# seanrjohnson/protein_gibbs_sampler

Hardware: AMD Instinct MI355X
Metric: sampled positions/sec (whole node), ESM-1b L=256 B=256 Gibbs (higher is better)
Workload: dtype bf16; 1 GPU; ESM_sampler ESM-1b (33 layers, d=1280) Gibbs: 256 chains in total, 256 per GPU x L=256 (T=258), P=25 positions per chain per iteration, mask=True top_k=0 temperature=1.0 burnin=inf; bf16 MFMA operands, fp32 accumulate + fp32 residual stream; synthetic weights N(0,0.025), embeddings N(0,0.3), LayerNorm jitter 0.1 (logit std ~10); global_batch=256, seq_len=256, parallelism=chains sharded 1-way (contiguous blocks), 1 RCCL all-gather at the end, n_layers=33

## Files before the change

protein_gibbs_sampler_amd/csrc/api_dbg.hip:

```cpp
#include <math.h>
#include <string.h>

#include <algorithm>
#include <vector>

#include "engine.h"
#include "gemm_epilogue.h"

using namespace pg;

namespace {
struct Dbg {
  int prev = -1;
  bool bad = false;
  std::vector<void*> bufs;
  Dbg() { (void)hipGetDevice(&prev); }
  ~Dbg() {
    for (void* p : bufs) (void)hipFree(p);
    if (prev >= 0) (void)hipSetDevice(prev);
  }
  int open(int device) {
    int n = 0;
    if (hipGetDeviceCount(&n) != hipSuccess || n == 0) return fail(PG_ERR_NO_DEVICE, "no HIP device visible");
    if (device < 0 || device >= n) return fail(PG_ERR_INVALID, "bad device ordinal");
// ... 83 lines not shown
  for (int i = 0; i < iters; ++i)
    if ((rc = launch())) return rc;
  PG_HIP(hipEventRecord(ev.b, nullptr));
  PG_HIP(hipEventSynchronize(ev.b));
  float ms = 0;
  PG_HIP(hipEventElapsedTime(&ms, ev.a, ev.b));
  *avg_ms = ms / iters;
  return PG_OK;
}
void dbg_noted_text(char* plan, int plan_bytes) {
  if (plan && plan_bytes > 0) snprintf(plan, (size_t)plan_bytes, "%s", noted_kernels().c_str());
}

template <typename Launch>
int dbg_attention_run(Dbg& s, int precision, bool strict, const float* qkv, float* ctx, int64_t M, int d, const int32_t* tok, char* plan,
                      int plan_bytes, Launch&& launch) {
  const float* dq = s.up(qkv, (size_t)M * 3 * d);
  const int32_t* dtok = s.up(tok, (size_t)M);
  bf16_t* bq = strict ? nullptr : s.alloc<bf16_t>((size_t)M * 3 * d);
  bf16_t* out = s.alloc<bf16_t>((size_t)M * d * (strict ? 3 : 1));
  float* wide = strict ? nullptr : s.alloc<float>((size_t)M * d);
  int rc = s.check();
  if (rc) return rc;
  clear_noted_kernels();
  if (!strict && (rc = to16(precision, dq, bq, M * 3 * d))) return rc;
  if ((rc = launch(dq, bq, out, dtok))) return rc;
  dbg_noted_text(plan, plan_bytes);
  return strict ? split3_rows_to_host(out, ctx, M, d) : down16(s, precision, out, wide, ctx, M * d);
}
}

extern "C" {

int pg_dbg_gemm(int device, int precision, const float* x, const float* w, const float* bias, float* out, int M, int N,
                int K, int epi) {
  return pg_dbg_gemm_v(device, precision, x, w, bias, out, M, N, K, epi, -1, -1, M, nullptr, 0);
}

int pg_dbg_gemm_v(int device, int precision, const float* x, const float* w, const float* bias, float* out, int M, int N, int K, int epi,
                  int variant, int have_ws, int m_live, char* plan, int plan_bytes) {
  if (plan && plan_bytes > 0) plan[0] = 0;
  int rc = dbg_precision("pg_dbg_gemm", precision, true);
  if (rc) return rc;
// ... 110 lines not shown
  }, iters, avg_ms);
}

int pg_dbg_gemm_plan(int M, int N, int K, int epi, int variant, int have_ws, int m_live, int n_cu, char* buf, int buf_bytes) {
  if (!buf || buf_bytes < 2 || M < 1 || N < 1 || K < 1 || n_cu < 1) return fail(PG_ERR_INVALID, "pg_dbg_gemm_plan: bad argument");
  std::string text;
  gemm_plan_text(M, N, K, epi, variant, have_ws != 0, m_live, n_cu, &text);
  snprintf(buf, (size_t)buf_bytes, "%s", text.c_str());
  return PG_OK;
}

int pg_dbg_attention_plan(int kind, int precision, int64_t n_seq_or_B, int T_or_C, int R, int H, int head_dim, int has_pad, int has_bias,
                          int row_step, int order_bh, int n_cu, char* buf, int buf_bytes) {
  const int rc = dbg_precision("pg_dbg_attention_plan", precision, true);
  if (rc) return rc;
  if (!buf || buf_bytes < 2 || (kind != 0 && kind != 1) || n_seq_or_B < 1 || H < 1 || n_cu < 1 || (kind == 1 && (R < 1 || n_seq_or_B > 0x7fffffff)))
    return fail(PG_ERR_INVALID, "pg_dbg_attention_plan: bad argument");
  const bool strict = precision == PG_PREC_FP32;
  std::string text;
  if (kind == 0 && strict) attention_f32_plan_text(n_seq_or_B, T_or_C, H, head_dim, has_pad != 0, has_bias != 0, row_step, &text);
  else if (kind == 0) attention_plan_text(n_seq_or_B, T_or_C, H, head_dim, has_pad != 0, has_bias != 0, row_step, n_cu, &text);
  else if (strict) msa_row_f32_plan_text((int)n_seq_or_B, R, T_or_C, H, has_pad != 0, &text);
  else msa_row_plan_text((int)n_seq_or_B, R, T_or_C, H, order_bh, &text);
  snprintf(buf, (size_t)buf_bytes, "%s", text.c_str());
  return PG_OK;
}

int pg_dbg_rowln_bench(int device, int M, int K, int iters, double* ms, double* max_diff) {
  if (!ms || M < 256 || K % 64 || K < 128 || iters < 1) return fail(PG_ERR_INVALID, "pg_dbg_rowln_bench: bad argument");
  Dbg d;
  int rc = d.open(device);
  if (rc) return rc;
  const int N = 768, Mp = round_up(M, kRowPad);
  const size_t n_f = (size_t)std::max(Mp, N) * std::max(K, N);
  const std::vector<float> hbuf = lcg_uniform(n_f + 5, 4242u);
// ... 115 lines not shown
  if ((rc = s.open(device))) return rc;
  const int d = H * head_dim;
  const bool strict = precision == PG_PREC_FP32;
  float* bias32 = bias_k ? s.alloc<float>((size_t)2 * d) : nullptr;
  if (bias_k) s.put(bias32, bias_k, (size_t)d), s.put(bias32 + d, bias_v, (size_t)d);
  bf16_t* bias16 = bias_k && !strict ? s.alloc<bf16_t>((size_t)2 * d) : nullptr;
  return dbg_attention_run(s, precision, strict, qkv, ctx, (int64_t)B * T, d, key_tok, plan, plan_bytes,
                           [&](const float* dq, const bf16_t* bq, bf16_t* out, const int32_t* dtok) {
    const SeqLayout chain = {1, T, 0, 1};
    if (strict) return launch_attention_f32(nullptr, dq, out, d, B, T, H, 3 * d, 3 * d, d, 2 * d, chain, dtok, pad_idx, bias32, head_dim);
    const int rc16 = bias_k ? to16(precision, bias32, bias16, 2 * d) : PG_OK;
    return rc16 ? rc16 : OPS(launch_attention_bf16, nullptr, bq, out, B, T, H, 3 * d, d, d, 2 * d, dtok, pad_idx, bias16, head_dim);
  });
}

int pg_dbg_layernorm_operand(int device, int precision, const float* x, const float* gamma, const float* beta, float* y, int M, int d,
                             float eps) {
  int rc = dbg_precision("pg_dbg_layernorm_operand", precision, true);
  if (rc) return rc;
  if (!x || !gamma || !beta || !y || M < 1 || d < 32 || d % 32) return fail(PG_ERR_INVALID, "pg_dbg_layernorm_operand: bad argument");
  Dbg s;
  if ((rc = s.open(device))) return rc;
  const bool split = precision == PG_PREC_FP32;
  const float* dx = s.up(x, (size_t)M * d);
  const float* dg = s.up(gamma, (size_t)d);
  const float* dbt = s.up(beta, (size_t)d);
  float* dy = s.alloc<float>((size_t)M * d);
  bf16_t* h = s.alloc<bf16_t>((size_t)M * d * (split ? 3 : 1));
  if ((rc = s.check())) return rc;
  if ((rc = OPS(launch_layernorm_bf16, nullptr, dx, dg, dbt, h, M, d, eps, split, 0, 0, true))) return rc;
// ... 261 lines not shown
```

protein_gibbs_sampler_amd/csrc/attention.hip:

```cpp
#include <stdlib.h>

#include "attn_frag.h"

PG_OPS_BEGIN


#ifdef PG_ATT_PROF
__device__ unsigned long long* pg_att_prof;
#define PG_T(slot, i)                                                                                              \
  do {                                                                                                             \
    if ((slot) < 8 && (threadIdx.x & 63) == 0)                                                                     \
      pg_att_prof[(((size_t)blockIdx.x * 4 + (threadIdx.x >> 6)) * 8 + (slot)) * 8 + (i)] = __builtin_readcyclecounter(); \
  } while (0)
#else
#define PG_T(slot, i)
#endif

constexpr int attention_occupancy(int maxkb, int hd, bool pad = false) {
  return hd == 128 ? (maxkb <= 8 || (maxkb == 10 && !pad) ? 2 : 1) : hd == 64 ? (maxkb <= 18 ? 2 : 1) : 2;
}
constexpr int attention_resident(int kb, int hd) {
  return hd == 128 ? (kb <= 4 ? 4 : (kb <= 6 ? 3 : (kb <= 10 ? 2 : 1))) : hd == 64 ? (kb <= 20 ? 2 : 1) : (kb <= 20 ? 4 : (kb <= 26 ? 3 : 2));
}
template <int MAXKB, bool PADMASK, bool BIASKV = false, bool SPLIT = false, int HD = 64>
__global__ __launch_bounds__(256, attention_occupancy(MAXKB, HD, PADMASK)) void attention_kernel(const bf16_t* __restrict__ qkv, bf16_t* __restrict__ ctx, int T,
                                                       int H, int ld_qkv_, int ld_ctx_, int k_off, int v_off,
                                                       SeqLayout sl, const int32_t* __restrict__ key_tok, int pad_idx,
                                                       const bf16_t* __restrict__ bias_kv, int split_from = 0, int split = 1) {
  constexpr int ROW = HD * 2, NKK = HD / 32, NDB = HD / 16;
  __shared__ __attribute__((aligned(16))) char smem[2 * MAXKB * 16 * ROW + (PADMASK ? MAXKB * 16 : 0)];
  char* Ks = smem;
  char* Vs = smem + MAXKB * 16 * ROW;
  char* padf = smem + 2 * MAXKB * 16 * ROW;

  const int tid = threadIdx.x, lane = tid & 63, wave = tid >> 6;
  PG_T(7, 0);
  int pair = blockIdx.x, qb_first = wave, qb_step = 4;
  if (SPLIT && (int)blockIdx.x >= split_from) {
    const int u = blockIdx.x - split_from;
    pair = split_from + u / split;
    qb_first = u % split + split * wave;
    qb_step = 4 * split;
  }
// ... 2 lines not shown
  const size_t ld_qkv = (size_t)ld_qkv_ * sl.row_step, ld_ctx = (size_t)ld_ctx_ * sl.row_step;
  const bf16_t* base = qkv + row0 * ld_qkv_ + h * HD;
  const int Tk = T + (BIASKV ? 1 : 0);
  constexpr int nkc = MAXKB / 2;

  stage_kv<MAXKB * 16, 256, BIASKV, HD>(Ks, Vs, tid, base, ld_qkv, k_off, v_off, 0, T, bias_kv + h * HD, bias_kv + (H + h) * HD);
  if (PADMASK) {
    for (int key = tid; key < MAXKB * 16; key += 256)
      padf[key] = (key < T && key_tok[row0 + (size_t)key * sl.row_step] == pad_idx) ? 1 : 0;
  }
  PG_T(7, 1);
  __syncthreads();
  PG_T(7, 2);

  const int fr = lane & 15, fq = lane >> 4;
  const int nqb = (T + 15) >> 4;
  bf16x8 qf[NKK], qn[NKK];
  auto load_q = [&](int qb, bf16x8 (&dst)[NKK]) {
    int qrow = qb * 16 + fr;
    if (qrow >= T) qrow = T - 1;
#pragma unroll
    for (int kk = 0; kk < NKK; ++kk) dst[kk] = *(const bf16x8*)(base + (size_t)qrow * ld_qkv + kk * 32 + fq * 8);
  };
  if (qb_first < nqb) load_q(qb_first, qf);
  for (int qb = qb_first; qb < nqb; qb += qb_step) {
    if (qb + qb_step < nqb) load_q(qb + qb_step, qn);
    PG_T(qb >> 2, 0);

    f32x4 st[MAXKB];
    {
      constexpr int CH = HD == 128 ? 2 : (MAXKB % 6 == 0) ? 6 : (MAXKB % 4 == 0 ? 4 : 2);
      bf16x8 kbuf[2][CH][NKK];
      auto load_chunk = [&](int ch, bf16x8 (&dst)[CH][NKK]) {
#pragma unroll
        for (int u = 0; u < CH; ++u) {
#if defined(PG_ATT_PROF) && PG_ATT_ABL == 1
          const int krow = (ch * CH + (u > 0 ? 0 : u)) * 16 + fr;
// ... 65 lines not shown
      };
      load_v(0, vbuf[0]);
      if (nkc > 1) load_v(1, vbuf[1]);
#pragma unroll
      for (int c = 0; c < nkc; ++c) {
        if (c + 2 < nkc) load_v(c + 2, vbuf[(c + 2) % 3]);
        const bf16x8 pf = p_frag(st[2 * c], st[2 * c + 1]);
        __builtin_amdgcn_sched_barrier(0);
#pragma unroll
        for (int db = 0; db < NDB; ++db) o[db] = mfma_op16(vbuf[c % 3][db].v, pf, o[db]);
        __builtin_amdgcn_sched_barrier(0);
      }
    }
    PG_T(qb >> 2, 3);
    const int q = qb * 16 + fr;
    if (q < T) store_ctx(o, inv, ctx + row0 * ld_ctx_ + (size_t)q * ld_ctx + h * HD + fq * 4);
    qf[0] = qn[0];
    if constexpr (NKK == 2) qf[1] = qn[1];
    if constexpr (NKK == 4) { qf[1] = qn[1]; qf[2] = qn[2]; qf[3] = qn[3]; }
    PG_T(qb >> 2, 4);
  }
  PG_T(7, 3);
}

template <int MAXKB, int OCC, bool PADMASK, bool BIASKV, int HD = 64>
__global__ __launch_bounds__(256, OCC) void attention_long_kernel(const bf16_t* __restrict__ qkv, bf16_t* __restrict__ ctx, int T,
                                                               int H, int ld_qkv_, int ld_ctx_, int k_off, int v_off,
                                                               SeqLayout sl, int n_qchunk, const int32_t* __restrict__ key_tok_,
                                                               int pad_idx, const bf16_t* __restrict__ bias_kv_) {
  const int32_t* __restrict__ key_tok = PADMASK ? key_tok_ : nullptr;
  const bf16_t* __restrict__ bias_kv = BIASKV ? bias_kv_ : nullptr;
// ... 178 lines not shown

int launch_attention_seq_bf16(hipStream_t s, const bf16_t* qkv, bf16_t* ctx, int64_t n_seq, int T, int H, int ld_qkv,
                              int ld_ctx, int k_off, int v_off, SeqLayout sl, const int32_t* key_tok, int pad_idx,
                              const bf16_t* bias_kv, int head_dim) {
  const AttentionPlan p = plan_attention(n_seq, T, H, head_dim, key_tok != nullptr, bias_kv != nullptr, sl.row_step, device_cu_count());
  if (!p.error.empty()) return fail(1, p.error);
  if (!p.grid) return 0;
  note_kernel(plan_text(p).c_str());
  auto launch = [&](auto hd) {
    constexpr int HD = decltype(hd)::value;
    if (!p.whole)
      return launch_long<HD>(p.pad, p.bias, dim3(p.grid), s, qkv, ctx, T, H, ld_qkv, ld_ctx, k_off, v_off, sl, p.n_qchunk, key_tok,
                             pad_idx, bias_kv);
    visit_rung(p.kb, [&](auto kb) {
      launch_rung<decltype(kb)::value, HD>(p.pad, p.bias, p.split > 1, dim3(p.grid), s, qkv, ctx, T, H, ld_qkv, ld_ctx, k_off, v_off,
                                           sl, key_tok, pad_idx, bias_kv, p.split_from, p.split);
    });
  };
  if (head_dim == 64) launch(std::integral_constant<int, 64>{});
  else if (head_dim == 128) launch(std::integral_constant<int, 128>{});
  else launch(std::integral_constant<int, 32>{});
  PG_HIP(hipGetLastError());
  return 0;
}

int launch_attention_bf16(hipStream_t s, const bf16_t* qkv, bf16_t* ctx, int B, int T, int H, int ld_qkv, int ld_ctx,
                          int k_off, int v_off, const int32_t* key_tok, int pad_idx, const bf16_t* bias_kv, int head_dim) {
  SeqLayout sl = {1, T, 0, 1};
  return launch_attention_seq_bf16(s, qkv, ctx, B, T, H, ld_qkv, ld_ctx, k_off, v_off, sl, key_tok, pad_idx, bias_kv, head_dim);
}

PG_OPS_END
```

protein_gibbs_sampler_amd/csrc/engine.h:

```cpp
#pragma once
#include <map>
#include <string>
#include <vector>

#include "kernels.h"

namespace pg {

#define OPS(fn, ...) (precision == PG_PREC_F16 ? opf16::fn(__VA_ARGS__) : opbf16::fn(__VA_ARGS__))

struct DevBuf {
  void* p = nullptr;
  size_t bytes = 0;
  int ensure(size_t need, hipStream_t s);
  void release();
  template <typename T> T* as() const { return (T*)p; }
};

struct Prof {
  struct Rec { int cls; hipEvent_t a, b; std::string kernels; };
  bool on = false;
  std::vector<Rec> recs;
  std::vector<hipEvent_t> pool;
  size_t used = 0;
// ... 32 lines not shown
  pg_model_config cfg;
  int device = 0;
  int precision = 0;
  hipStream_t own_stream = nullptr, stream = nullptr;
  std::vector<void*> owned;

  float *embed = nullptr, *pos = nullptr, *msa_pos = nullptr, *embed_out = nullptr;
  float embed_scale() const { return cfg.arch == PG_ARCH_ESM1 ? sqrtf((float)cfg.d_model) : 1.0f; }
  LnW ln_before, ln_after, head_ln;
  DenseW head_dense;
  float* head_bias = nullptr;
  std::vector<EsmLayer> esm_layers;
  std::vector<MsaLayer> msa_layers;

  DevBuf x, h, qkv, ctx, ffn, sel_h, sel_g, logits, d_tokens, d_idx, d_samp_tok, d_samp_logits, d_rowmap, scratch;
  DevBuf x_sel, ctx_sel, h_sel, ffn_sel;
  int resid_gemm_ln(const bf16_t* a, const DenseW& W, float* x, int M_rows, int64_t M_real, int lda, const LnW& ln, bf16_t* h,
                    float* ws = nullptr, size_t ws_bytes = 0, int prof_class = PC_GEMM, int colmajor_R = 0, int colmajor_C = 0);
  DevBuf tmp_idx, tmp_out;
  DevBuf splitk;
  bool esm_pad_in_batch = false;
  float* splitk_ws(int rows, int n, int K, int64_t batch_rows);
  int64_t job_items = 0;
  int64_t order_items = 0;
  int64_t job_batch(int64_t B) const { return order_items > 0 ? order_items : (job_items > B ? job_items : B); }
  int64_t batch_rows_for(int64_t B, int64_t rows_per_item) const { return job_batch(B) * rows_per_item; }
  int64_t batch_rows = 0;
  int sel_gemm_rows(int64_t n_sel, int64_t Np) const;
  DevBuf d_iter;
  PgChainLayerW* chain_layers = nullptr;
  DevBuf chain_sync, chain_part;
// ... 26 lines not shown
  int rope_rows = 0;
  int rope(void* qkv_rows, int64_t M, int T);
  int dense3(const bf16_t* x3, const DenseW& W, float* out, int Mp, bool accumulate);
  int dense3_gelu(const bf16_t* x3, const DenseW& W, int Mp, const DenseW* next = nullptr);
  bool dense3_wants_dup(const DenseW& W, int Mp, bool gelu = false) const;
  Prof prof;

  ~Engine();
  int init(const pg_model_config* c, const pg_tensor* tensors, int n_tensors, int device_ordinal, int precision);

  int size_activations(int64_t Mp);
  int ffn_block(const DenseW& out, const FfnW& F, const LnW* next_ln, int Mi, int64_t M);
  int ffn_strict(const FfnW& F, int Mi, int64_t M);
  bool prune_last(int64_t n_draws, int64_t token_rows) const;
  int pruned_tail(const DenseW& out, const FfnW& F, const int32_t* sel_idx, const int32_t* sel_row_map, int P, int width, int64_t n_sel,
                  const int32_t* d_iter, int Ni, bool ln_in_gemm);
  int esm_trunk(const int32_t* d_tok, int B, int T, const int32_t* sel_idx, int P, int64_t n_sel, const int32_t* d_iter);
  int head(const int32_t* d_idx, const int32_t* d_row_map, int P, int width, int64_t n_sel, float* d_logits,
           const float* x_src = nullptr);
  int trunk(const int32_t* d_tok, int B, int R, int C, const int32_t* sel_idx = nullptr, const int32_t* sel_row_map = nullptr, int P = 0,
            int64_t n_sel = 0, const int32_t* d_iter = nullptr);
  int masked_logits(int32_t* d_tok, int B, int R, int C, const int32_t* idx, const int32_t* mask_map, const int32_t* sel_map,
                    int64_t n_rows, int P, bool mask, int mask_idx, float* lg, const int32_t* dit = nullptr);
  int esm_gibbs_device(int32_t* d_tok, int B, int T, const int32_t* d_idx, int n_iters, int P, const pg_sample_params* sp,
                       float* d_samp_logits, int32_t* d_samp_tok);
  int msa_trunk(const int32_t* d_tok, int B, int R, int C, const int32_t* sel_idx, const int32_t* sel_row_map, int P, int64_t n_sel);
  int msa_gibbs_device(int32_t* d_tok, int B, int R, int C, const int32_t* d_idx, int n_iters, int P,
                       const pg_sample_params* sp, float* d_samp_logits, int32_t* d_samp_tok);
  int msa_single_device(int32_t* d_tok, int B, int R, int C, int mask_row, int target_row, const int32_t* d_step_idx,
                        const int32_t* step_sample_flag_host, int n_steps, int P_max, const pg_sample_params* sp,
                        float* d_samp_logits, int32_t* d_samp_tok);
// ... 17 lines not shown
```

protein_gibbs_sampler_amd/csrc/engine.hip:

```cpp
#include <algorithm>

#include "engine.h"

#include <math.h>
#include <stdlib.h>
#include <string.h>

#include "gemm_epilogue.h"

namespace pg {

static thread_local std::string g_last_error;
void set_error(const std::string& msg) { g_last_error = msg; }
int fail(int code, const std::string& msg) {
  g_last_error = msg;
  return code;
}
const char* last_error_cstr() { return g_last_error.c_str(); }

static thread_local std::string g_noted;
void note_kernel(const char* label, long tiles, int splits) {
  if (g_noted.size() > 512) return;
  if (!g_noted.empty()) g_noted += " + ";
  g_noted += label;
// ... 60 lines not shown
  if (it == m.end()) {
    err = "missing tensor '" + name + "'";
    return nullptr;
  }
  if (it->second->numel != numel) {
    err = "tensor '" + name + "' has " + std::to_string(it->second->numel) + " elements, expected " + std::to_string(numel);
    return nullptr;
  }
  return it->second->data;
}

Engine::~Engine() {
  if (device >= 0) (void)hipSetDevice(device);
  for (void* p : owned) (void)hipFree(p);
  DevBuf* bufs[] = {&x, &h, &qkv, &ctx, &ffn, &sel_h, &sel_g, &logits, &d_tokens, &d_idx, &d_samp_tok, &d_samp_logits,
                    &d_rowmap, &scratch, &d_iter, &tmp_idx, &tmp_out, &x_sel, &ctx_sel, &h_sel, &ffn_sel, &ffn_f32, &scores, &splitk,
                    &chain_sync, &chain_part, &chain_snap};
  for (DevBuf* b : bufs) b->release();
  if (chain_err) (void)hipHostFree(chain_err);
  if (range_err) (void)hipHostFree(range_err);
  prof.destroy();
  if (graph_exec) (void)hipGraphExecDestroy(graph_exec);
  if (own_stream) (void)hipStreamDestroy(own_stream);
}

namespace {
struct Uploader {
  Engine* e;
  const TensorMap* tm;
  const int precision;
  std::string err;
// ... 339 lines not shown
  return dense3(ffn.as<bf16_t>(), F.fc2, X, Mi, true);
}

int Engine::ffn_block(const DenseW& out, const FfnW& F, const LnW* next_ln, int Mi, int64_t M) {
  const int d = cfg.d_model, f = cfg.d_ffn;
  float* X = x.as<float>();
  bf16_t* Hh = h.as<bf16_t>();
  bf16_t* FFN = ffn.as<bf16_t>();
  int rc;
  if ((rc = resid_gemm_ln(ctx.as<bf16_t>(), out, X, Mi, M, d, F.ln, Hh, nullptr, 0, PC_GEMM_OUT))) return rc;
  if ((rc = timed(PC_GEMM_FC1, [&] { return OPS(launch_gemm_bf16, stream, Hh, F.fc1.w, F.fc1.b, FFN, Mi, f, d, d, d, f, EPI_BF16_GELU, nullptr, 0, (int)M); }))) return rc;
  if (next_ln) return resid_gemm_ln(FFN, F.fc2, X, Mi, M, f, *next_ln, Hh, splitk_ws(Mi, d, f, batch_rows), splitk.bytes, PC_GEMM_FC2);
  return timed(PC_GEMM_FC2, [&] { return OPS(launch_gemm_bf16, stream, FFN, F.fc2.w, F.fc2.b, X, Mi, d, f, f, f, d, EPI_F32_RESID, splitk_ws(Mi, d, f, batch_rows), splitk.bytes, (int)M); });
}

bool Engine::prune_last(int64_t n_draws, int64_t token_rows) const {
  static const int prune = env_int("PGIBBS_PRUNE_LAST", 1);
  return prune && !strict() && n_draws > 0 && 2 * n_draws < token_rows;
}

int Engine::pruned_tail(const DenseW& out, const FfnW& F, const int32_t* sel_idx, const int32_t* sel_row_map, int P, int width,
                        int64_t n_sel, const int32_t* d_iter_, int Ni, bool ln_in_gemm) {
  const int d = cfg.d_model, f = cfg.d_ffn;
  const float eps = cfg.layer_norm_eps;
  const int64_t Np = round_up64(n_sel, kRowPad);
  int rc;
  if ((rc = x_sel.ensure((size_t)Np * d * 4, stream)) || (rc = ctx_sel.ensure((size_t)Np * d * 2, stream)) ||
      (rc = h_sel.ensure((size_t)Np * d * 2, stream)) || (rc = ffn_sel.ensure((size_t)Np * f * 2, stream))) return rc;
  float* XS = x_sel.as<float>();
  bf16_t* FS = ffn_sel.as<bf16_t>();
  rc = timed(PC_HEAD, [&] {
    int r2 = launch_gather_rows(stream, x.as<float>(), XS, sel_idx, sel_row_map, P, width, n_sel, d * 4, d_iter_);
    if (r2) return r2;
    return launch_gather_rows(stream, ctx.as<bf16_t>(), ctx_sel.as<bf16_t>(), sel_idx, sel_row_map, P, width, n_sel, d * 2, d_iter_);
  });
  if (rc) return rc;
  if ((rc = timed(PC_GEMM, [&] { return OPS(launch_gemm_bf16, stream, ctx_sel.as<bf16_t>(), out.w, out.b, XS, Ni, d, d, d, d, d, EPI_F32_RESID); }))) return rc;
  if (ln_in_gemm && gemm_ln_skinny_ok(Ni, f, d)) {
    if ((rc = timed(PC_GEMM, [&] { return OPS(launch_gemm_ln_skinny, stream, XS, d, F.ln.g, F.ln.b, eps, F.fc1.w, F.fc1.b, FS, Ni, f, d, d, f, EPI_BF16_GELU); }))) return rc;
  } else {
    if ((rc = timed(PC_LN, [&] { return OPS(launch_layernorm_bf16, stream, XS, F.ln.g, F.ln.b, h_sel.as<bf16_t>(), n_sel, d, eps); }))) return rc;
    if ((rc = timed(PC_GEMM, [&] { return OPS(launch_gemm_bf16, stream, h_sel.as<bf16_t>(), F.fc1.w, F.fc1.b, FS, Ni, f, d, d, d, f, EPI_BF16_GELU); }))) return rc;
  }
  return timed(PC_GEMM, [&] { return OPS(launch_gemm_bf16, stream, FS, F.fc2.w, F.fc2.b, XS, Ni, d, f, f, f, d, EPI_F32_RESID, splitk_ws(Ni, d, f, batch_rows), splitk.bytes); });
}

int Engine::trunk(const int32_t* d_tok, int B, int R, int C, const int32_t* sel_idx, const int32_t* sel_row_map, int P, int64_t n_sel,
                  const int32_t* d_iter_) {
// ... 54 lines not shown
    if (rc == kChainTrunkUnfit) {
      chain_disabled = true;
    } else if (rc) {
      return rc;
    } else {
      static const int fault_at = env_int("PGIBBS_CHAIN_TRUNK_FAULT", 0);
      static int launches = 0;
      if (fault_at > 0 && ++launches == fault_at) *chain_err = 1;
      if (!sel_idx) return PG_OK;
      l_first = cfg.n_layers - 1;
      attn_done = true;
    }
  }
  for (int l = l_first; l < cfg.n_layers; ++l) {
    const EsmLayer& L = esm_layers[l];
    if (attn_done) {
    } else if (ln_in_gemm) {
      if ((rc = timed(PC_GEMM, [&] { return OPS(launch_gemm_ln_skinny, stream, X, d, L.ln1.g, L.ln1.b, eps, L.qkv.w, L.qkv.b, QKV, Mi, 3 * d, d, d, 3 * d, EPI_BF16); }))) return rc;
    } else {
      if ((rc = timed(PC_GEMM_QKV, [&] { return OPS(launch_gemm_bf16, stream, Hh, L.qkv.w, L.qkv.b, QKV, Mi, 3 * d, d, d, d, 3 * d, EPI_BF16); }))) return rc;
    }
    if (!attn_done && (rc = rope(QKV, M, T))) return rc;
    if (!attn_done)
      if ((rc = timed(PC_ATTN, [&] { return OPS(launch_attention_bf16, stream, QKV, CTX, B, T, cfg.n_heads, 3 * d, d, d, 2 * d, esm_pad_in_batch ? d_tok : nullptr, cfg.pad_idx, L.bias_kv16, head_dim); }))) return rc;
    const bool last = l == cfg.n_layers - 1;
    if (sel_idx && last) return pruned_tail(L.out, L.ffn, sel_idx, nullptr, P, T, n_sel, d_iter_, sel_gemm_rows(n_sel, round_up64(n_sel, kRowPad)), ln_in_gemm);
    if (!ln_in_gemm) {
      if ((rc = ffn_block(L.out, L.ffn, last ? nullptr : &esm_layers[l + 1].ln1, Mi, M))) return rc;
      continue;
    }
    const FfnW& F = L.ffn;
    if ((rc = timed(PC_GEMM, [&] { return OPS(launch_gemm_bf16, stream, CTX, L.out.w, L.out.b, X, Mi, d, d, d, d, d, EPI_F32_RESID); }))) return rc;
    if ((rc = timed(PC_GEMM, [&] { return OPS(launch_gemm_ln_skinny, stream, X, d, F.ln.g, F.ln.b, eps, F.fc1.w, F.fc1.b, FFN, Mi, f, d, d, f, EPI_BF16_GELU); }))) return rc;
    if ((rc = timed(PC_GEMM, [&] { return OPS(launch_gemm_bf16, stream, FFN, F.fc2.w, F.fc2.b, X, Mi, d, f, f, f, d, EPI_F32_RESID, splitk_ws(Mi, d, f, batch_rows), splitk.bytes, (int)M); }))) return rc;
  }
  return PG_OK;
}

int Engine::resid_gemm_ln(const bf16_t* a, const DenseW& W, float* x, int M_rows, int64_t M_real, int lda, const LnW& ln, bf16_t* h,
                          float* ws, size_t ws_bytes, int prof_class, int colmajor_R, int colmajor_C) {
// ... 308 lines not shown
```

protein_gibbs_sampler_amd/csrc/kernels_ops.inc:

```
int launch_gemm_bf16(hipStream_t s, const bf16_t* X, const bf16_t* W, const float* bias, void* out, int M, int N, int K,
                     int ldx, int ldw, int ldo, int epi, float* ws = nullptr, size_t ws_bytes = 0, int m_live = 0);
int gemm_splitk_splits(int K);
size_t gemm_splitk_ws_bytes(int M, int N, int K);
int launch_gemm_bf16_variant(hipStream_t s, const bf16_t* X, const bf16_t* W, const float* bias, void* out, int M, int N,
                             int K, int ldx, int ldw, int ldo, int epi, int variant, float* ws = nullptr, size_t ws_bytes = 0,
                             int m_live = 0);

bool gemm_ln_skinny_ok(int M, int N, int K);
int launch_gemm_ln_skinny(hipStream_t s, const float* X, int ldx, const float* gamma, const float* beta, float eps, const bf16_t* W,
                          const float* bias, void* out, int M, int N, int K, int ldw, int ldo, int epi, int nb_force = 0);
bool chain_trunk_ok(int M, int d_model, int d_ffn, int n_heads);
size_t chain_trunk_sync_bytes();
size_t chain_trunk_part_bytes(int M, int d_model);
int launch_chain_trunk(hipStream_t s, const PgChainTrunkArgs& a, int M, int d_model);
int launch_gemm_big(hipStream_t s, const bf16_t* X, const bf16_t* W, const float* bias, void* out, int M, int N, int K, int ldx,
                    int ldw, int ldo, int epi, int m_live = 0);
bool gemm_ladder_has(int epi, int h);
int launch_gemm_ladder(hipStream_t s, const bf16_t* X, const bf16_t* W, const float* bias, void* out, int m_live, int m_rows, int h,
                       int N, int K, int ldx, int ldw, int ldo, int epi);
bool gemm_rowln_ok(int m_rows, int N, int K);
int launch_gemm_rowln(hipStream_t s, const bf16_t* A, const bf16_t* W, const float* bias, float* x, const float* gamma,
                      const float* beta, bf16_t* h, int m_live, int m_rows, int K, int lda, int ldw, float eps, int colmajor_R = 0,
                      int colmajor_C = 0, int abl = 0);
void gemm_plan_text(int M, int N, int K, int epi, int variant, bool have_ws, int m_live, int n_cu, std::string* text);
void gemm_big_geometry(int M, int N, int K, int* m_main_panels, int* tail_rows);
int launch_gemm_w16(hipStream_t s, const bf16_t* X, const bf16_t* W, const float* bias, void* out, int M, int N, int K, int ldx,
                    int ldw, int ldo, int epi, int abl = 0, int tail_rows = 0);
int launch_gemm_split3(hipStream_t s, const bf16_t* X3, const bf16_t* W3, const float* bias, void* out, int M, int N, int K, int ldo,
                       int epi);
bool gemm_split3_fused(int M, int N, int K, int epi);
int launch_gemm_split3_w16(hipStream_t s, const bf16_t* X3, const bf16_t* W3, const float* bias, void* out, int M, int N, int K,
                           int ldo, int epi);

int launch_attention_bf16(hipStream_t s, const bf16_t* qkv, bf16_t* ctx, int B, int T, int H, int ld_qkv, int ld_ctx,
                          int k_off, int v_off, const int32_t* key_tok = nullptr, int pad_idx = -1, const bf16_t* bias_kv = nullptr,
                          int head_dim = 64);
int launch_attention_seq_bf16(hipStream_t s, const bf16_t* qkv, bf16_t* ctx, int64_t n_seq, int T, int H, int ld_qkv,
                              int ld_ctx, int k_off, int v_off, SeqLayout sl, const int32_t* key_tok = nullptr,
                              int pad_idx = -1, const bf16_t* bias_kv = nullptr, int head_dim = 64);
size_t msa_row_split_scratch_bytes(int B, int R, int C, int H, int order_bh);
void attention_plan_text(int64_t n_seq, int T, int H, int head_dim, bool has_pad, bool has_bias, int row_step, int n_cu, std::string* text);
void attention_f32_plan_text(int64_t n_seq, int T, int H, int head_dim, bool has_pad, bool has_bias, int row_step, std::string* text);
void msa_row_plan_text(int B, int R, int C, int H, int order_bh, std::string* text);
void msa_row_f32_plan_text(int B, int R, int C, int H, bool has_pad, std::string* text);
int launch_msa_row_attention_bf16(hipStream_t s, const bf16_t* qkv, bf16_t* ctx, int B, int R, int C, int H, int ld_qkv,
                                  int ld_ctx, int k_off, int v_off, float scale, float* partial = nullptr,
                                  size_t partial_bytes = 0, int order_bh = 0);

int launch_embed_ln(hipStream_t s, const int32_t* tokens, const float* embed, const float* pos, const float* msa_pos,
                    const float* gamma, const float* beta, float* x, int64_t n_tok, int T, int d, int pad_idx,
                    int mask_idx, int token_dropout, int rows_per_msa, float eps,
                    const float* gamma2 = nullptr, const float* beta2 = nullptr, bf16_t* h2 = nullptr,
                    float embed_scale = 1.0f);
int launch_rope(hipStream_t s, void* qkv, bool f32, const float* table, int table_rows, int64_t M, int T, int H, int ld,
// ... 36 lines not shown
```

Before: 69750 sampled positions/s.

## Prune last-layer query projection and attention to sampled positions only

In the final ESM layer, only the K/V projection is computed for all tokens. The Q projection and attention run only for the P gathered sampled rows, using a new SEL variant of the attention kernel that reads gathered queries. This removes the Q-third of the last QKV GEMM and most of the last attention work for unsampled rows. The cost is extra gather and launch steps, plus a small skinny GEMM. The path is on by default through PGIBBS_PRUNE_LAST=2 and applies only when ESM-1b runs with no pad mask and no bias_kv.

```diff
diff --git a/include/pgibbs_dbg.h b/include/pgibbs_dbg.h
--- /dev/null
+++ b/include/pgibbs_dbg.h
@@ -0,0 +1,17 @@
+#ifndef PGIBBS_DBG_H
+#define PGIBBS_DBG_H
+
+#include "pgibbs.h"
+
+#ifdef __cplusplus
+extern "C" {
+#endif
+
+int pg_dbg_attention_sel(int device, int precision, const float* qkv, const int32_t* idx, int B, int T, int H, int head_dim, int P,
+                         float* ctx_sel);
+
+#ifdef __cplusplus
+}
+#endif
+
+#endif
diff --git a/protein_gibbs_sampler_amd/csrc/api_dbg.hip b/protein_gibbs_sampler_amd/csrc/api_dbg.hip
--- a/protein_gibbs_sampler_amd/csrc/api_dbg.hip
+++ b/protein_gibbs_sampler_amd/csrc/api_dbg.hip
@@ -6,6 +6,7 @@
 
 #include "engine.h"
 #include "gemm_epilogue.h"
+#include "pgibbs_dbg.h"
 
 using namespace pg;
 
@@ -121,19 +122,20 @@
 
 template <typename Launch>
 int dbg_attention_run(Dbg& s, int precision, bool strict, const float* qkv, float* ctx, int64_t M, int d, const int32_t* tok, char* plan,
-                      int plan_bytes, Launch&& launch) {
+                      int plan_bytes, Launch&& launch, int64_t out_rows = 0) {
+  const int64_t Mo = out_rows > 0 ? out_rows : M;
   const float* dq = s.up(qkv, (size_t)M * 3 * d);
   const int32_t* dtok = s.up(tok, (size_t)M);
   bf16_t* bq = strict ? nullptr : s.alloc<bf16_t>((size_t)M * 3 * d);
-  bf16_t* out = s.alloc<bf16_t>((size_t)M * d * (strict ? 3 : 1));
-  float* wide = strict ? nullptr : s.alloc<float>((size_t)M * d);
+  bf16_t* out = s.alloc<bf16_t>((size_t)Mo * d * (strict ? 3 : 1));
+  float* wide = strict ? nullptr : s.alloc<float>((size_t)Mo * d);
   int rc = s.check();
   if (rc) return rc;
   clear_noted_kernels();
   if (!strict && (rc = to16(precision, dq, bq, M * 3 * d))) return rc;
   if ((rc = launch(dq, bq, out, dtok))) return rc;
   dbg_noted_text(plan, plan_bytes);
-  return strict ? split3_rows_to_host(out, ctx, M, d) : down16(s, precision, out, wide, ctx, M * d);
+  return strict ? split3_rows_to_host(out, ctx, Mo, d) : down16(s, precision, out, wide, ctx, Mo * d);
 }
 }
 
@@ -274,11 +276,14 @@
                           int row_step, int order_bh, int n_cu, char* buf, int buf_bytes) {
   const int rc = dbg_precision("pg_dbg_attention_plan", precision, true);
   if (rc) return rc;
-  if (!buf || buf_bytes < 2 || (kind != 0 && kind != 1) || n_seq_or_B < 1 || H < 1 || n_cu < 1 || (kind == 1 && (R < 1 || n_seq_or_B > 0x7fffffff)))
+  if (!buf || buf_bytes < 2 || kind < 0 || kind > 2 || n_seq_or_B < 1 || H < 1 || n_cu < 1 || (kind == 1 && (R < 1 || n_seq_or_B > 0x7fffffff)) ||
+      (kind == 2 && R < 1))
     return fail(PG_ERR_INVALID, "pg_dbg_attention_plan: bad argument");
   const bool strict = precision == PG_PREC_FP32;
   std::string text;
-  if (kind == 0 && strict) attention_f32_plan_text(n_seq_or_B, T_or_C, H, head_dim, has_pad != 0, has_bias != 0, row_step, &text);
+  if (kind == 2 && strict) text = "declined: the strict mode";
+  else if (kind == 2) attention_sel_plan_text(n_seq_or_B, T_or_C, H, head_dim, R, has_pad != 0, has_bias != 0, &text);
+  else if (kind == 0 && strict) attention_f32_plan_text(n_seq_or_B, T_or_C, H, head_dim, has_pad != 0, has_bias != 0, row_step, &text);
   else if (kind == 0) attention_plan_text(n_seq_or_B, T_or_C, H, head_dim, has_pad != 0, has_bias != 0, row_step, n_cu, &text);
   else if (strict) msa_row_f32_plan_text((int)n_seq_or_B, R, T_or_C, H, has_pad != 0, &text);
   else msa_row_plan_text((int)n_seq_or_B, R, T_or_C, H, order_bh, &text);
@@ -424,6 +429,30 @@
   });
 }
 
+int pg_dbg_attention_sel(int device, int precision, const float* qkv, const int32_t* idx, int B, int T, int H, int head_dim, int P,
+                         float* ctx_sel) {
+  int rc = dbg_precision("pg_dbg_attention_sel", precision, false);
+  if (rc) return rc;
+  if (!qkv || !idx || !ctx_sel || B < 1 || T < 1 || H < 1 || P < 1) return fail(PG_ERR_INVALID, "pg_dbg_attention_sel: bad argument");
+  if ((double)B * T * 3 * H * head_dim > 2147483647.0) return fail(PG_ERR_INVALID, "pg_dbg_attention_sel: more than 2^31 - 1 qkv values");
+  std::string text;
+  OPS(attention_sel_plan_text, B, T, H, head_dim, P, false, false, &text);
+  if (text.compare(0, 4, "sel ") != 0) return fail(PG_ERR_INVALID, "pg_dbg_attention_sel: " + text);
+  const int64_t n_sel = (int64_t)B * P;
+  for (int64_t r = 0; r < n_sel; ++r)
+    if (idx[r] < 0 || idx[r] >= T) return fail(PG_ERR_INVALID, "pg_dbg_attention_sel: idx must be in 0 ... T - 1");
+  Dbg s;
+  if ((rc = s.open(device))) return rc;
+  const int d = H * head_dim;
+  const int32_t* di = s.up(idx, (size_t)n_sel);
+  bf16_t* qs = s.alloc<bf16_t>((size_t)n_sel * 3 * d);
+  return dbg_attention_run(s, precision, false, qkv, ctx_sel, (int64_t)B * T, d, nullptr, nullptr, 0,
+                           [&](const float*, const bf16_t* bq, bf16_t* out, const int32_t*) {
+    const int rg = launch_gather_rows(nullptr, bq, qs, di, nullptr, P, T, n_sel, 3 * d * 2);
+    return rg ? rg : OPS(launch_attention_sel_bf16, nullptr, bq, qs, out, B, T, H, P, 3 * d, 3 * d, d, d, 2 * d, head_dim);
+  }, n_sel);
+}
+
 int pg_dbg_layernorm_operand(int device, int precision, const float* x, const float* gamma, const float* beta, float* y, int M, int d,
                              float eps) {
   int rc = dbg_precision("pg_dbg_layernorm_operand", precision, true);
diff --git a/protein_gibbs_sampler_amd/csrc/attention.hip b/protein_gibbs_sampler_amd/csrc/attention.hip
--- a/protein_gibbs_sampler_amd/csrc/attention.hip
+++ b/protein_gibbs_sampler_amd/csrc/attention.hip
@@ -22,11 +22,13 @@
 constexpr int attention_resident(int kb, int hd) {
   return hd == 128 ? (kb <= 4 ? 4 : (kb <= 6 ? 3 : (kb <= 10 ? 2 : 1))) : hd == 64 ? (kb <= 20 ? 2 : 1) : (kb <= 20 ? 4 : (kb <= 26 ? 3 : 2));
 }
-template <int MAXKB, bool PADMASK, bool BIASKV = false, bool SPLIT = false, int HD = 64>
+template <int MAXKB, bool PADMASK, bool BIASKV = false, bool SPLIT = false, int HD = 64, bool SEL = false>
 __global__ __launch_bounds__(256, attention_occupancy(MAXKB, HD, PADMASK)) void attention_kernel(const bf16_t* __restrict__ qkv, bf16_t* __restrict__ ctx, int T,
                                                        int H, int ld_qkv_, int ld_ctx_, int k_off, int v_off,
                                                        SeqLayout sl, const int32_t* __restrict__ key_tok, int pad_idx,
-                                                       const bf16_t* __restrict__ bias_kv, int split_from = 0, int split = 1) {
+                                                       const bf16_t* __restrict__ bias_kv, int split_from = 0, int split = 1,
+                                                       const bf16_t* __restrict__ q_sel = nullptr, int ld_q = 0, int P = 0) {
+  static_assert(!SEL || (!PADMASK && !BIASKV && !SPLIT), "the gathered-query form is built without <pad> mask, bias key and split");
   constexpr int ROW = HD * 2, NKK = HD / 32, NDB = HD / 16;
   __shared__ __attribute__((aligned(16))) char smem[2 * MAXKB * 16 * ROW + (PADMASK ? MAXKB * 16 : 0)];
   char* Ks = smem;
@@ -59,13 +61,20 @@
   PG_T(7, 2);
 
   const int fr = lane & 15, fq = lane >> 4;
-  const int nqb = (T + 15) >> 4;
+  const int nqb = ((SEL ? P : T) + 15) >> 4;
   bf16x8 qf[NKK], qn[NKK];
   auto load_q = [&](int qb, bf16x8 (&dst)[NKK]) {
     int qrow = qb * 16 + fr;
-    if (qrow >= T) qrow = T - 1;
-#pragma unroll
-    for (int kk = 0; kk < NKK; ++kk) dst[kk] = *(const bf16x8*)(base + (size_t)qrow * ld_qkv + kk * 32 + fq * 8);
+    if constexpr (SEL) {
+      if (qrow >= P) qrow = P - 1;
+      const bf16_t* qsrc = q_sel + ((size_t)seq * P + qrow) * ld_q + h * HD;
+#pragma unroll
+      for (int kk = 0; kk < NKK; ++kk) dst[kk] = *(const bf16x8*)(qsrc + kk * 32 + fq * 8);
+    } else {
+      if (qrow >= T) qrow = T - 1;
+#pragma unroll
+      for (int kk = 0; kk < NKK; ++kk) dst[kk] = *(const bf16x8*)(base + (size_t)qrow * ld_qkv + kk * 32 + fq * 8);
+    }
   };
   if (qb_first < nqb) load_q(qb_first, qf);
   for (int qb = qb_first; qb < nqb; qb += qb_step) {
@@ -161,7 +170,11 @@
     }
     PG_T(qb >> 2, 3);
     const int q = qb * 16 + fr;
-    if (q < T) store_ctx(o, inv, ctx + row0 * ld_ctx_ + (size_t)q * ld_ctx + h * HD + fq * 4);
+    if constexpr (SEL) {
+      if (q < P) store_ctx(o, inv, ctx + ((size_t)seq * P + q) * ld_ctx_ + h * HD + fq * 4);
+    } else {
+      if (q < T) store_ctx(o, inv, ctx + row0 * ld_ctx_ + (size_t)q * ld_ctx + h * HD + fq * 4);
+    }
     qf[0] = qn[0];
     if constexpr (NKK == 2) qf[1] = qn[1];
     if constexpr (NKK == 4) { qf[1] = qn[1]; qf[2] = qn[2]; qf[3] = qn[3]; }
@@ -370,7 +383,7 @@
                              pad_idx, bias_kv);
     visit_rung(p.kb, [&](auto kb) {
       launch_rung<decltype(kb)::value, HD>(p.pad, p.bias, p.split > 1, dim3(p.grid), s, qkv, ctx, T, H, ld_qkv, ld_ctx, k_off, v_off,
-                                           sl, key_tok, pad_idx, bias_kv, p.split_from, p.split);
+                                           sl, key_tok, pad_idx, bias_kv, p.split_from, p.split, (const bf16_t*)nullptr, 0, 0);
     });
   };
   if (head_dim == 64) launch(std::integral_constant<int, 64>{});
@@ -386,4 +399,61 @@
   return launch_attention_seq_bf16(s, qkv, ctx, B, T, H, ld_qkv, ld_ctx, k_off, v_off, sl, key_tok, pad_idx, bias_kv, head_dim);
 }
 
+struct AttentionSelPlan {
+  std::string declined;
+  int kb = 0, hd = 64, nqb = 0;
+  unsigned grid = 0;
+};
+
+static AttentionSelPlan plan_attention_sel(int64_t n_seq, int T, int H, int head_dim, int P, bool has_pad, bool has_bias) {
+  AttentionSelPlan p;
+  p.hd = head_dim;
+  auto decline = [&](const std::string& why) { p.declined = why; return p; };
+  const std::string head_err = attention_head_error(head_dim, has_bias);
+  if (!head_err.empty()) return decline(head_err);
+  if (has_pad) return decline("a <pad> key mask");
+  if (has_bias) return decline("the bias_k / bias_v key");
+  if (n_seq < 1 || T < 1 || H < 1 || P < 1) return decline("an empty shape");
+  if (n_seq * H > 0x7fffffff || n_seq * P > 0x7fffffff) return decline("too many sequences");
+  static const int whole128 = env_int("PGIBBS_ATTN_HD128_WHOLE", 1);
+  p.kb = head_dim == 128 && !whole128 ? 0 : attention_rung(T, attention_fine_ladder(), attention_max_keys(head_dim));
+  if (!p.kb) return decline("more keys than a whole-sequence rung holds");
+  p.nqb = (P + 15) / 16;
+  p.grid = (unsigned)(n_seq * H);
+  return p;
+}
+
+static std::string plan_text(const AttentionSelPlan& p) {
+  if (!p.declined.empty()) return "declined: " + p.declined;
+  return "sel kb" + std::to_string(p.kb) + " hd" + std::to_string(p.hd) + " nqb" + std::to_string(p.nqb) + " " + std::to_string(p.grid) + "wg";
+}
+void attention_sel_plan_text(int64_t n_seq, int T, int H, int head_dim, int P, bool has_pad, bool has_bias, std::string* text) {
+  *text = plan_text(plan_attention_sel(n_seq, T, H, head_dim, P, has_pad, has_bias));
+}
+bool attention_sel_ok(int64_t n_seq, int T, int H, int head_dim, int P, bool has_pad, bool has_bias) {
+  return plan_attention_sel(n_seq, T, H, head_dim, P, has_pad, has_bias).declined.empty();
+}
+
+int launch_attention_sel_bf16(hipStream_t s, const bf16_t* qkv, const bf16_t* q_sel, bf16_t* ctx_sel, int64_t n_seq, int T, int H, int P,
+                              int ld_qkv, int ld_q, int ld_ctx, int k_off, int v_off, int head_dim) {
+  const AttentionSelPlan p = plan_attention_sel(n_seq, T, H, head_dim, P, false, false);
+  if (!p.declined.empty()) return fail(1, "attention with gathered queries: " + p.declined);
+  note_kernel(plan_text(p).c_str());
+  const SeqLayout sl = {1, T, 0, 1};
+  auto launch = [&](auto hd) {
+    constexpr int HD = decltype(hd)::value;
+    visit_rung(p.kb, [&](auto kb) {
+      constexpr int KB = decltype(kb)::value;
+      if constexpr (KB * 16 <= attention_max_keys(HD))
+        hipLaunchKernelGGL((attention_kernel<KB, false, false, false, HD, true>), dim3(p.grid), dim3(256), 0, s, qkv, ctx_sel, T, H,
+                           ld_qkv, ld_ctx, k_off, v_off, sl, (const int32_t*)nullptr, -1, (const bf16_t*)nullptr, 0, 1, q_sel, ld_q, P);
+    });
+  };
+  if (head_dim == 64) launch(std::integral_constant<int, 64>{});
+  else if (head_dim == 128) launch(std::integral_constant<int, 128>{});
+  else launch(std::integral_constant<int, 32>{});
+  PG_HIP(hipGetLastError());
+  return 0;
+}
+
 PG_OPS_END
diff --git a/protein_gibbs_sampler_amd/csrc/engine.h b/protein_gibbs_sampler_amd/csrc/engine.h
--- a/protein_gibbs_sampler_amd/csrc/engine.h
+++ b/protein_gibbs_sampler_amd/csrc/engine.h
@@ -70,7 +70,7 @@
   std::vector<MsaLayer> msa_layers;
 
   DevBuf x, h, qkv, ctx, ffn, sel_h, sel_g, logits, d_tokens, d_idx, d_samp_tok, d_samp_logits, d_rowmap, scratch;
-  DevBuf x_sel, ctx_sel, h_sel, ffn_sel;
+  DevBuf x_sel, ctx_sel, h_sel, q_sel, ffn_sel;
   int resid_gemm_ln(const bf16_t* a, const DenseW& W, float* x, int M_rows, int64_t M_real, int lda, const LnW& ln, bf16_t* h,
                     float* ws = nullptr, size_t ws_bytes = 0, int prof_class = PC_GEMM, int colmajor_R = 0, int colmajor_C = 0);
   DevBuf tmp_idx, tmp_out;
@@ -127,7 +127,9 @@
   int ffn_strict(const FfnW& F, int Mi, int64_t M);
   bool prune_last(int64_t n_draws, int64_t token_rows) const;
   int pruned_tail(const DenseW& out, const FfnW& F, const int32_t* sel_idx, const int32_t* sel_row_map, int P, int width, int64_t n_sel,
-                  const int32_t* d_iter, int Ni, bool ln_in_gemm);
+                  const int32_t* d_iter, int Ni, bool ln_in_gemm, bool ctx_gathered = false);
+  bool prune_last_q(int B, int T, int P, int64_t n_sel, int Mi, bool has_bias) const;
+  int sel_qkv_attention(const EsmLayer& L, int B, int T, const int32_t* sel_idx, int P, int64_t n_sel, const int32_t* d_iter, int Mi);
   int esm_trunk(const int32_t* d_tok, int B, int T, const int32_t* sel_idx, int P, int64_t n_sel, const int32_t* d_iter);
   int head(const int32_t* d_idx, const int32_t* d_row_map, int P, int width, int64_t n_sel, float* d_logits,
            const float* x_src = nullptr);
diff --git a/protein_gibbs_sampler_amd/csrc/engine.hip b/protein_gibbs_sampler_amd/csrc/engine.hip
--- a/protein_gibbs_sampler_amd/csrc/engine.hip
+++ b/protein_gibbs_sampler_amd/csrc/engine.hip
@@ -98,7 +98,7 @@
   if (device >= 0) (void)hipSetDevice(device);
   for (void* p : owned) (void)hipFree(p);
   DevBuf* bufs[] = {&x, &h, &qkv, &ctx, &ffn, &sel_h, &sel_g, &logits, &d_tokens, &d_idx, &d_samp_tok, &d_samp_logits,
-                    &d_rowmap, &scratch, &d_iter, &tmp_idx, &tmp_out, &x_sel, &ctx_sel, &h_sel, &ffn_sel, &ffn_f32, &scores, &splitk,
+                    &d_rowmap, &scratch, &d_iter, &tmp_idx, &tmp_out, &x_sel, &ctx_sel, &h_sel, &q_sel, &ffn_sel, &ffn_f32, &scores, &splitk,
                     &chain_sync, &chain_part, &chain_snap};
   for (DevBuf* b : bufs) b->release();
   if (chain_err) (void)hipHostFree(chain_err);
@@ -468,13 +468,38 @@
   return timed(PC_GEMM_FC2, [&] { return OPS(launch_gemm_bf16, stream, FFN, F.fc2.w, F.fc2.b, X, Mi, d, f, f, f, d, EPI_F32_RESID, splitk_ws(Mi, d, f, batch_rows), splitk.bytes, (int)M); });
 }
 
+static int prune_level() {
+  static const int level = env_int("PGIBBS_PRUNE_LAST", 2);
+  return level;
+}
+
 bool Engine::prune_last(int64_t n_draws, int64_t token_rows) const {
-  static const int prune = env_int("PGIBBS_PRUNE_LAST", 1);
-  return prune && !strict() && n_draws > 0 && 2 * n_draws < token_rows;
+  return prune_level() && !strict() && n_draws > 0 && 2 * n_draws < token_rows;
+}
+
+bool Engine::prune_last_q(int B, int T, int P, int64_t n_sel, int Mi, bool has_bias) const {
+  const int d = cfg.d_model;
+  return prune_level() >= 2 && !esm2() && Mi > 48 && d % 64 == 0 && n_sel == (int64_t)B * P &&
+         OPS(attention_sel_ok, B, T, cfg.n_heads, head_dim, P, esm_pad_in_batch, has_bias);
+}
+
+int Engine::sel_qkv_attention(const EsmLayer& L, int B, int T, const int32_t* sel_idx, int P, int64_t n_sel, const int32_t* d_iter_, int Mi) {
+  const int d = cfg.d_model;
+  const int64_t M = (int64_t)B * T, Np = round_up64(n_sel, kRowPad);
+  int rc;
+  if ((rc = h_sel.ensure((size_t)Np * d * 2, stream)) || (rc = q_sel.ensure((size_t)Np * d * 2, stream)) ||
+      (rc = ctx_sel.ensure((size_t)Np * d * 2, stream))) return rc;
+  bf16_t* Hh = h.as<bf16_t>();
+  bf16_t* QKV = qkv.as<bf16_t>();
+  if ((rc = timed(PC_GEMM_QKV, [&] { return OPS(launch_gemm_bf16, stream, Hh, L.qkv.w + (size_t)d * d, L.qkv.b + d, QKV + d, Mi, 2 * d, d, d, d, 3 * d, EPI_BF16, nullptr, 0, (int)M); }))) return rc;
+  if ((rc = timed(PC_HEAD, [&] { return launch_gather_rows(stream, Hh, h_sel.as<bf16_t>(), sel_idx, nullptr, P, T, n_sel, d * 2, d_iter_); }))) return rc;
+  const int Nq = std::max(sel_gemm_rows(n_sel, Np), 64);
+  if ((rc = timed(PC_GEMM_QKV, [&] { return OPS(launch_gemm_bf16, stream, h_sel.as<bf16_t>(), L.qkv.w, L.qkv.b, q_sel.as<bf16_t>(), Nq, d, d, d, d, d, EPI_BF16); }))) return rc;
+  return timed(PC_ATTN, [&] { return OPS(launch_attention_sel_bf16, stream, QKV, q_sel.as<bf16_t>(), ctx_sel.as<bf16_t>(), B, T, cfg.n_heads, P, 3 * d, d, d, d, 2 * d, head_dim); });
 }
 
 int Engine::pruned_tail(const DenseW& out, const FfnW& F, const int32_t* sel_idx, const int32_t* sel_row_map, int P, int width,
-                        int64_t n_sel, const int32_t* d_iter_, int Ni, bool ln_in_gemm) {
+                        int64_t n_sel, const int32_t* d_iter_, int Ni, bool ln_in_gemm, bool ctx_gathered) {
   const int d = cfg.d_model, f = cfg.d_ffn;
   const float eps = cfg.layer_norm_eps;
   const int64_t Np = round_up64(n_sel, kRowPad);
@@ -485,7 +510,7 @@
   bf16_t* FS = ffn_sel.as<bf16_t>();
   rc = timed(PC_HEAD, [&] {
     int r2 = launch_gather_rows(stream, x.as<float>(), XS, sel_idx, sel_row_map, P, width, n_sel, d * 4, d_iter_);
-    if (r2) return r2;
+    if (r2 || ctx_gathered) return r2;
     return launch_gather_rows(stream, ctx.as<bf16_t>(), ctx_sel.as<bf16_t>(), sel_idx, sel_row_map, P, width, n_sel, d * 2, d_iter_);
   });
   if (rc) return rc;
@@ -570,6 +595,11 @@
   }
   for (int l = l_first; l < cfg.n_layers; ++l) {
     const EsmLayer& L = esm_layers[l];
+    const bool last = l == cfg.n_layers - 1;
+    if (sel_idx && last && !attn_done && !ln_in_gemm && prune_last_q(B, T, P, n_sel, Mi, L.bias_kv16 != nullptr)) {
+      if ((rc = sel_qkv_attention(L, B, T, sel_idx, P, n_sel, d_iter_, Mi))) return rc;
+      return pruned_tail(L.out, L.ffn, sel_idx, nullptr, P, T, n_sel, d_iter_, sel_gemm_rows(n_sel, round_up64(n_sel, kRowPad)), ln_in_gemm, true);
+    }
     if (attn_done) {
     } else if (ln_in_gemm) {
       if ((rc = timed(PC_GEMM, [&] { return OPS(launch_gemm_ln_skinny, stream, X, d, L.ln1.g, L.ln1.b, eps, L.qkv.w, L.qkv.b, QKV, Mi, 3 * d, d, d, 3 * d, EPI_BF16); }))) return rc;
@@ -579,7 +609,6 @@
     if (!attn_done && (rc = rope(QKV, M, T))) return rc;
     if (!attn_done)
       if ((rc = timed(PC_ATTN, [&] { return OPS(launch_attention_bf16, stream, QKV, CTX, B, T, cfg.n_heads, 3 * d, d, d, 2 * d, esm_pad_in_batch ? d_tok : nullptr, cfg.pad_idx, L.bias_kv16, head_dim); }))) return rc;
-    const bool last = l == cfg.n_layers - 1;
     if (sel_idx && last) return pruned_tail(L.out, L.ffn, sel_idx, nullptr, P, T, n_sel, d_iter_, sel_gemm_rows(n_sel, round_up64(n_sel, kRowPad)), ln_in_gemm);
     if (!ln_in_gemm) {
       if ((rc = ffn_block(L.out, L.ffn, last ? nullptr : &esm_layers[l + 1].ln1, Mi, M))) return rc;
diff --git a/protein_gibbs_sampler_amd/csrc/kernels_ops.inc b/protein_gibbs_sampler_amd/csrc/kernels_ops.inc
--- a/protein_gibbs_sampler_amd/csrc/kernels_ops.inc
+++ b/protein_gibbs_sampler_amd/csrc/kernels_ops.inc
@@ -38,6 +38,10 @@
 int launch_attention_seq_bf16(hipStream_t s, const bf16_t* qkv, bf16_t* ctx, int64_t n_seq, int T, int H, int ld_qkv,
                               int ld_ctx, int k_off, int v_off, SeqLayout sl, const int32_t* key_tok = nullptr,
                               int pad_idx = -1, const bf16_t* bias_kv = nullptr, int head_dim = 64);
+bool attention_sel_ok(int64_t n_seq, int T, int H, int head_dim, int P, bool has_pad, bool has_bias);
+void attention_sel_plan_text(int64_t n_seq, int T, int H, int head_dim, int P, bool has_pad, bool has_bias, std::string* text);
+int launch_attention_sel_bf16(hipStream_t s, const bf16_t* qkv, const bf16_t* q_sel, bf16_t* ctx_sel, int64_t n_seq, int T, int H, int P,
+                              int ld_qkv, int ld_q, int ld_ctx, int k_off, int v_off, int head_dim = 64);
 size_t msa_row_split_scratch_bytes(int B, int R, int C, int H, int order_bh);
 void attention_plan_text(int64_t n_seq, int T, int H, int head_dim, bool has_pad, bool has_bias, int row_step, int n_cu, std::string* text);
 void attention_f32_plan_text(int64_t n_seq, int T, int H, int head_dim, bool has_pad, bool has_bias, int row_step, std::string* text);
```

Result: no change. 69950 sampled positions/s (median of 6 runs) (+0.3%).
